# sourmash-bio/sourmash

Measured on AMD Instinct MI355X. Metric: Gbase/s sketched (k=31, scaled=1000), higher is better.
Workload: dtype u64; 1 GPU; C2: sketch synthetic random DNA resident in HBM as ASCII, per GPU 1000 records of 10000000 bases (10000000000 bases, 10000001000 bytes with their separators), k=31 scaled=1000 seed=42; one step = k-mer kernel + radix sort + unique; records_per_gpu=1000, record_len=10000000, bases_per_gpu=10000000000, bytes_per_gpu=10000001000, ksize=31, scaled=1000, unique_hashes_rank0=9998668, unique_hashes_job=9998668, collectives=none (the exchange runs with --full)

## Files before the change

sourmash_amd/csrc/sketch.hip:

```cpp
#include <hip/hip_runtime.h>
#include <stdint.h>
#include <stdlib.h>
#include <utility>
#include "kmer_core.hpp"
#include "sketch_kernel.hpp"
#include "device_api.hpp"

namespace smg {

constexpr int GENERIC_MAX_K = 256;
constexpr int GENERIC_TILE = 4096;

__global__ __launch_bounds__(SK_BLOCK) void sketch_dna_generic_kernel(
    const uint8_t* __restrict__ seq, uint64_t len, uint32_t k, uint64_t seed, uint64_t thr,
    uint64_t* __restrict__ out, unsigned long long* __restrict__ out_count, uint64_t out_cap, uint64_t n_tiles,
    int dense) {
    __shared__ uint8_t s_in[GENERIC_TILE + GENERIC_MAX_K];
    for (uint64_t tile = blockIdx.x; tile < n_tiles; tile += gridDim.x) {
        const uint64_t base = tile * (uint64_t)GENERIC_TILE;
        __syncthreads();
        for (uint32_t i = threadIdx.x; i < GENERIC_TILE + k - 1; i += SK_BLOCK)
            s_in[i] = (base + i < len) ? seq[base + i] : 0;
        __syncthreads();
        for (uint32_t p = threadIdx.x; p < GENERIC_TILE; p += SK_BLOCK) {
            uint8_t fwd[GENERIC_MAX_K], rev[GENERIC_MAX_K];
            bool ok = true;
            for (uint32_t j = 0; j < k; ++j) {
                const uint8_t u = s_in[p + j] & 0xdf;
                uint8_t c;
                switch (u) {
                case 'A': c = 'T'; break;
                case 'C': c = 'G'; break;
                case 'G': c = 'C'; break;
                case 'T': c = 'A'; break;
                default: c = 0; ok = false;
                }
                fwd[j] = u;
                rev[k - 1 - j] = c;
            }
            if (!ok) continue;
            bool use_rev = false;
            for (uint32_t j = 0; j < k; ++j) {
                if (fwd[j] != rev[j]) { use_rev = rev[j] < fwd[j]; break; }
            }
            const uint64_t h = mmh3_h1_bytes(use_rev ? rev : fwd, k, seed);
            if ((h - 1) < thr) {
                if (dense) {
                    if (base + p < out_cap) out[base + p] = h;
                } else {
                    const unsigned long long g = atomicAdd(out_count, 1ull);
                    if (g < out_cap) out[g] = h;
                }
            }
        }
    }
}

__global__ __launch_bounds__(SK_BLOCK) void first_invalid_kernel(const uint8_t* __restrict__ seq, uint64_t len,
                                                                unsigned long long* __restrict__ first) {
    unsigned long long best = ~0ull;
    for (uint64_t i = (uint64_t)blockIdx.x * SK_BLOCK + threadIdx.x; i < len; i += (uint64_t)gridDim.x * SK_BLOCK) {
        const uint8_t u = seq[i] & 0xdf;
        if (!(u == 'A' || u == 'C' || u == 'G' || u == 'T')) { best = i; break; }
    }
    if (best != ~0ull) atomicMin(first, best);
}

constexpr int FAST_MAX_K = SK_FAST_MAX_K;
constexpr int FAST_HERE_K = 64;

static hipError_t sketch_any(const uint8_t* d_seq, uint64_t len, uint32_t k, uint64_t seed, uint64_t thr,
                             uint64_t* d_out, unsigned long long* d_count, uint64_t cap, bool dense,
                             hipStream_t stream) {
    if (len < k || k == 0) return hipSuccess;
    static const bool generic_only = [] { const char* e = getenv("SMG_SKETCH_GENERIC"); return e && *e == '1'; }();
    constexpr uint32_t words_from = (uint32_t)FAST_MAX_K + 1u;
    if (k >= words_from && !generic_only) return sketch_dna_words_launch(d_seq, len, k, seed, thr, d_out, d_count, cap, dense, stream);
    if (!dense && k <= (uint32_t)FAST_MAX_K && !generic_only) {
        const sketch_launch_fn f = k <= (uint32_t)FAST_HERE_K ? sparse_launcher_from<0>(k, std::make_integer_sequence<int, FAST_HERE_K>())
                                                             : sparse_launcher_long(k);
        return f(d_seq, len, seed, thr, d_out, d_count, cap, false, stream);
    }
    if (dense && k <= (uint32_t)FAST_MAX_K && !generic_only)
        return dense_launcher(k)(d_seq, len, seed, thr, d_out, d_count, cap, true, stream);
    if (!generic_only || k > (uint32_t)GENERIC_MAX_K) return sketch_dna_words_launch(d_seq, len, k, seed, thr, d_out, d_count, cap, dense, stream);
    const uint64_t n_tiles = (len + GENERIC_TILE - 1) / GENERIC_TILE;
    const uint64_t max_blocks = 256ull * 8;
    const unsigned grid = (unsigned)(n_tiles < max_blocks ? n_tiles : max_blocks);
    hipLaunchKernelGGL(sketch_dna_generic_kernel, dim3(grid), dim3(SK_BLOCK), 0, stream, d_seq, len, k, seed, thr,
                       d_out, d_count, cap, n_tiles, dense ? 1 : 0);
    return hipGetLastError();
}

hipError_t sketch_dna_launch(const uint8_t* d_seq, uint64_t len, uint32_t k, uint64_t seed, uint64_t thr,
                             uint64_t* d_out, unsigned long long* d_count, uint64_t cap, hipStream_t stream) {
    return sketch_any(d_seq, len, k, seed, thr, d_out, d_count, cap, false, stream);
}

hipError_t kmer_hashes_launch(const uint8_t* d_seq, uint64_t len, uint32_t k, uint64_t seed, uint64_t* d_out,
                              uint64_t n_kmers, hipStream_t stream) {
    return sketch_any(d_seq, len, k, seed, ~0ull, d_out, nullptr, n_kmers, true, stream);
}

hipError_t first_invalid_launch(const uint8_t* d_seq, uint64_t len, unsigned long long* d_first, hipStream_t stream) {
    if (len == 0) return hipSuccess;
    const uint64_t nb = (len + SK_BLOCK - 1) / SK_BLOCK;
    const unsigned grid = (unsigned)(nb < 2048 ? nb : 2048);
    hipLaunchKernelGGL(first_invalid_kernel, dim3(grid), dim3(SK_BLOCK), 0, stream, d_seq, len, d_first);
    return hipGetLastError();
}

}
```

sourmash_amd/csrc/sketch_kernel.hpp:

```cpp
#pragma once
#include <hip/hip_runtime.h>
#include <stdint.h>
#include <utility>
#include "kmer_core.hpp"

namespace smg {

constexpr int SK_BLOCK = 256;
constexpr int SK_FAST_MAX_K = 88;
constexpr int sk_part_size(int first_k_minus_1) { return SK_FAST_MAX_K - first_k_minus_1 < 16 ? SK_FAST_MAX_K - first_k_minus_1 : 16; }
constexpr int SK_OUT_CAP = 2048;

constexpr bool sk_plain_mul(int k, bool dense) {
    if (dense) return k == 1 || k == 5 || k == 8 || k == 25 || k == 28 || k == 81 || k == 82 || k == 84;
    return k == 50 || k == 51;
}

template <int K, int P, bool DENSE>
__global__ __launch_bounds__(SK_BLOCK) void sketch_dna_kernel(
    const uint8_t* __restrict__ seq, uint64_t len, uint64_t seed, uint64_t thr,
    uint64_t* __restrict__ out, unsigned long long* __restrict__ out_count, uint64_t out_cap,
    uint64_t n_tiles, uint32_t skip) {
    using G = LaneGeom<K, P>;
    constexpr int TILE = SK_BLOCK * P;
    constexpr int LANE_RD = ((G::NW + 3) / 4) * 4;
    constexpr int IN_DW = (SK_BLOCK - 1) * (P / 4) + LANE_RD;
    constexpr int IN_CHUNKS = (IN_DW + 3) / 4;
    static_assert(P % 4 == 0, "lane runs must start dword aligned");

    __shared__ __attribute__((aligned(16))) uint32_t s_in[IN_CHUNKS * 4];
    __shared__ uint64_t s_out[SK_OUT_CAP];
    __shared__ unsigned int s_cnt;
    __shared__ unsigned long long s_base;

    const int tid = threadIdx.x;
    if (tid == 0) s_cnt = 0;

    for (uint64_t tile = blockIdx.x; tile < n_tiles; tile += gridDim.x) {
        const uint64_t base = tile * (uint64_t)TILE;
        __syncthreads();
        for (int c = tid; c < IN_CHUNKS; c += SK_BLOCK) {
            const uint64_t off = base + (uint64_t)c * 16;
            uint4 v = make_uint4(0, 0, 0, 0);
            if (off + 16 <= len) {
                v = *reinterpret_cast<const uint4*>(seq + off);
            } else if (off < len) {
                uint32_t w[4] = {0, 0, 0, 0};
                for (uint64_t b = off; b < len; ++b) w[(b - off) >> 2] |= (uint32_t)seq[b] << (8 * ((b - off) & 3));
                v = make_uint4(w[0], w[1], w[2], w[3]);
            }
            if (off == 0 && skip) {
                uint32_t w[4] = {v.x, v.y, v.z, v.w};
                for (uint32_t b = 0; b < skip; ++b) w[b >> 2] &= ~(0xffu << (8 * (b & 3)));
                v = make_uint4(w[0], w[1], w[2], w[3]);
            }
            *reinterpret_cast<uint4*>(&s_in[c * 4]) = v;
        }
        __syncthreads();
        uint32_t raw[LANE_RD];
        const uint4* wp = reinterpret_cast<const uint4*>(&s_in[tid * (P / 4)]);
        static_assert((P / 4) % 4 == 0 || P == 8 || P == 4, "window must stay 16-byte aligned for P=16,32");
#pragma unroll
        for (int i = 0; i < LANE_RD / 4; ++i) {
            if constexpr ((P / 4) % 4 == 0) {
                const uint4 v = wp[i];
                raw[4 * i] = v.x; raw[4 * i + 1] = v.y; raw[4 * i + 2] = v.z; raw[4 * i + 3] = v.w;
            } else {
                const uint32_t* p32 = &s_in[tid * (P / 4) + 4 * i];
                raw[4 * i] = p32[0]; raw[4 * i + 1] = p32[1]; raw[4 * i + 2] = p32[2]; raw[4 * i + 3] = p32[3];
            }
        }
        process_lane<K, P, !DENSE, sk_plain_mul(K, DENSE)>(raw, seed, thr, [&](int o, uint64_t h) {
            if constexpr (DENSE) {
                const uint64_t pos = base + (uint64_t)tid * P + (uint64_t)o - skip;
                if (pos < out_cap) out[pos] = h;
                return;
            }
            const unsigned int idx = atomicAdd(&s_cnt, 1u);
            if (idx < (unsigned)SK_OUT_CAP) {
                s_out[idx] = h;
            } else {
                const unsigned long long g = atomicAdd(out_count, 1ull);
                if (g < out_cap) out[g] = h;
            }
        });
        if constexpr (DENSE) continue;
        __syncthreads();
        const unsigned int cnt = s_cnt;
        if (cnt >= (unsigned)SK_OUT_CAP / 2) {
            const unsigned int n = cnt < (unsigned)SK_OUT_CAP ? cnt : (unsigned)SK_OUT_CAP;
            if (tid == 0) s_base = atomicAdd(out_count, (unsigned long long)n);
            __syncthreads();
            const unsigned long long b = s_base;
            for (unsigned int i = tid; i < n; i += SK_BLOCK)
                if (b + i < out_cap) out[b + i] = s_out[i];
            __syncthreads();
            if (tid == 0) s_cnt = 0;
        }
    }
    if constexpr (DENSE) return;
    __syncthreads();
    const unsigned int cnt = s_cnt;
    if (cnt) {
        const unsigned int n = cnt < (unsigned)SK_OUT_CAP ? cnt : (unsigned)SK_OUT_CAP;
        if (tid == 0) s_base = atomicAdd(out_count, (unsigned long long)n);
        __syncthreads();
        const unsigned long long b = s_base;
        for (unsigned int i = tid; i < n; i += SK_BLOCK)
            if (b + i < out_cap) out[b + i] = s_out[i];
    }
}


typedef hipError_t (*sketch_launch_fn)(const uint8_t*, uint64_t, uint64_t, uint64_t, uint64_t*, unsigned long long*, uint64_t, bool,
                                       hipStream_t);
template <int K>
static hipError_t launch_sparse_k(const uint8_t* d_seq, uint64_t len, uint64_t seed, uint64_t thr, uint64_t* d_out,
                                  unsigned long long* d_count, uint64_t cap, bool, hipStream_t stream) {
    constexpr uint64_t TILE = (uint64_t)SK_BLOCK * 16;
    const uint32_t skip = (uint32_t)((uintptr_t)d_seq & 15);
    d_seq -= skip;
    len += skip;
    const uint64_t n_tiles = (len + TILE - 1) / TILE;
    if (n_tiles == 0) return hipSuccess;
    const uint64_t max_blocks = 256ull * 8;
    const unsigned grid = (unsigned)(n_tiles < max_blocks ? n_tiles : max_blocks);
    hipLaunchKernelGGL((sketch_dna_kernel<K, 16, false>), dim3(grid), dim3(SK_BLOCK), 0, stream, d_seq, len, seed, thr, d_out,
                       d_count, cap, n_tiles, skip);
    return hipGetLastError();
}
template <int K0, int... KS>
static sketch_launch_fn sparse_launcher_from(uint32_t k, std::integer_sequence<int, KS...>) {
    static const sketch_launch_fn table[] = {&launch_sparse_k<K0 + KS + 1>...};
    return table[k - K0 - 1];
}
template <int K>
static hipError_t launch_dense_k(const uint8_t* d_seq, uint64_t len, uint64_t seed, uint64_t thr, uint64_t* d_out,
                                 unsigned long long* d_count, uint64_t cap, bool, hipStream_t stream) {
    constexpr uint64_t TILE = (uint64_t)SK_BLOCK * 16;
    const uint32_t skip = (uint32_t)((uintptr_t)d_seq & 15);
    d_seq -= skip;
    len += skip;
    const uint64_t n_tiles = (len + TILE - 1) / TILE;
    if (n_tiles == 0) return hipSuccess;
    const uint64_t max_blocks = 256ull * 8;
    const unsigned grid = (unsigned)(n_tiles < max_blocks ? n_tiles : max_blocks);
    hipLaunchKernelGGL((sketch_dna_kernel<K, 16, true>), dim3(grid), dim3(SK_BLOCK), 0, stream, d_seq, len, seed, thr, d_out,
                       d_count, cap, n_tiles, skip);
    return hipGetLastError();
}
template <int K0, int... KS>
static sketch_launch_fn dense_launcher_from(uint32_t k, std::integer_sequence<int, KS...>) {
    static const sketch_launch_fn table[] = {&launch_dense_k<K0 + KS + 1>...};
    return table[k - K0 - 1];
}
sketch_launch_fn dense_launcher_0(uint32_t k);
sketch_launch_fn dense_launcher_1(uint32_t k);
sketch_launch_fn dense_launcher_2(uint32_t k);
sketch_launch_fn dense_launcher_3(uint32_t k);
sketch_launch_fn dense_launcher_4(uint32_t k);
sketch_launch_fn dense_launcher_5(uint32_t k);
inline sketch_launch_fn dense_launcher(uint32_t k) {
    switch ((k - 1u) / 16u) {
    case 0: return dense_launcher_0(k);
    case 1: return dense_launcher_1(k);
    case 2: return dense_launcher_2(k);
    case 3: return dense_launcher_3(k);
    case 4: return dense_launcher_4(k);
    default: return dense_launcher_5(k);
    }
}
sketch_launch_fn sparse_launcher_long_0(uint32_t k);
sketch_launch_fn sparse_launcher_long_1(uint32_t k);
inline sketch_launch_fn sparse_launcher_long(uint32_t k) { return k <= 80u ? sparse_launcher_long_0(k) : sparse_launcher_long_1(k); }
static_assert(SK_FAST_MAX_K > 80 && SK_FAST_MAX_K <= 96, "the part tables above");

}
```

sourmash_amd/csrc/kmer_core.hpp:

```cpp
#pragma once
#include "murmur3.hpp"
#include <utility>

namespace smg {

SMG_HD uint32_t perm_b32(uint32_t hi, uint32_t lo, uint32_t sel) {
#if defined(__HIP_DEVICE_COMPILE__)
    return __builtin_amdgcn_perm(hi, lo, sel);
#else
    const uint64_t v = ((uint64_t)hi << 32) | lo;
    uint32_t r = 0;
    for (int i = 0; i < 4; ++i) {
        const uint32_t s = (sel >> (8 * i)) & 0xff;
        uint32_t b;
        if (s < 8) b = (uint32_t)(v >> (8 * s)) & 0xff;
        else if (s == 0x0c) b = 0;
        else b = 0xff;
        r |= b << (8 * i);
    }
    return r;
#endif
}

SMG_HD uint32_t alignbyte_b32(uint32_t hi, uint32_t lo, uint32_t n) {
#if defined(__HIP_DEVICE_COMPILE__)
    return __builtin_amdgcn_alignbyte(hi, lo, n);
#else
    return (uint32_t)((((uint64_t)hi << 32) | lo) >> (8 * n));
#endif
}

SMG_HD bool any_lane(bool p) {
#if defined(__HIP_DEVICE_COMPILE__)
    return __builtin_amdgcn_ballot_w64(p) != 0ull;
#else
    return p;
#endif
}

SMG_HD uint32_t bitselect(uint32_t mask, uint32_t b, uint32_t c) {
#if defined(__HIP_DEVICE_COMPILE__)
    return __builtin_amdgcn_bitop3_b32(mask, b, c, 0xCA);
#else
    return (mask & b) | (~mask & c);
#endif
}

SMG_HD uint32_t opaque(uint32_t x) {
#if defined(__HIP_DEVICE_COMPILE__)
    asm volatile("" : "+v"(x));
#endif
    return x;
}

SMG_HD uint32_t bswap32(uint32_t x) { return perm_b32(0u, x, 0x00010203u); }

constexpr uint32_t LUT_SELF = 'A' | ('C' << 8) | ('T' << 16) | ((uint32_t)'G' << 24);
constexpr uint32_t LUT_COMP = 'T' | ('G' << 8) | ('A' << 16) | ((uint32_t)'C' << 24);

template <int K, int P>
struct LaneGeom {
    static constexpr int NBYTES = P + K - 1;
    static constexpr int NW = (NBYTES + 3) / 4;
    static constexpr int NWK = (K + 3) / 4;
    static constexpr int NCH = (K + 7) / 8;
    static constexpr uint32_t LAST_MASK = (K % 4) ? ((1u << (8 * (K % 4))) - 1u) : 0xffffffffu;
};

constexpr uint32_t rev_sel(int a) {
    return (uint32_t)(a + 3) | ((uint32_t)(a + 2) << 8) | ((uint32_t)(a + 1) << 16) | ((uint32_t)a << 24);
}
constexpr uint32_t rev_sel_partial(int a, int nb) {
    uint32_t s = 0;
    for (int i = 0; i < 4; ++i) {
        const uint32_t b = (i < nb) ? (uint32_t)(a + nb - 1 - i) : 0x0cu;
        s |= b << (8 * i);
    }
    return s;
}

template <int K, int P, int O>
struct PosOps {
    using G = LaneGeom<K, P>;

    template <int D>
    static SMG_HD uint32_t fwd(const uint32_t* U) {
        constexpr int q = (O >> 2) + D, a = O & 3;
        uint32_t v;
        if constexpr (a == 0) v = U[q];
        else if constexpr (q + 1 < G::NW) v = alignbyte_b32(U[q + 1], U[q], a);
        else v = U[q] >> (8 * a);
        if constexpr (D == G::NWK - 1) v &= G::LAST_MASK;
        return v;
    }

    template <int D>
    static SMG_HD uint32_t rev(const uint32_t* C) {
        constexpr int nb = (K - 4 * D) >= 4 ? 4 : (K - 4 * D);
        constexpr int s = O + K - 4 * D - nb;
        constexpr int q = s >> 2, a = s & 3;
        constexpr uint32_t sel = (nb == 4) ? rev_sel(a) : rev_sel_partial(a, nb);
        if constexpr (q + 1 < G::NW) return perm_b32(C[q + 1], C[q], sel);
        else return perm_b32(0u, C[q], sel);
    }

    template <int CH>
    static SMG_HD uint64_t be_chunk(const uint32_t* W) {
        uint64_t v = (uint64_t)bswap32(W[2 * CH]) << 32;
        if constexpr (2 * CH + 1 < G::NWK) v |= bswap32(W[2 * CH + 1]);
        return v;
    }

    template <int CH>
    static SMG_HD uint64_t be_chunk_opaque(const uint32_t* W) {
        uint64_t v = (uint64_t)bswap32(opaque(W[2 * CH])) << 32;
        if constexpr (2 * CH + 1 < G::NWK) v |= bswap32(opaque(W[2 * CH + 1]));
        return v;
    }

    template <int CH>
    static SMG_HD void tie_break(const uint32_t* F, const uint32_t* R, bool& tie, bool& gt) {
        if constexpr (CH < G::NCH) {
            const uint64_t bf = be_chunk_opaque<CH>(F), br = be_chunk_opaque<CH>(R);
            gt = gt || (tie && bf > br);
            tie = tie && (bf == br);
            tie_break<CH + 1>(F, R, tie, gt);
        }
    }

    template <int... D>
    static SMG_HD void build(const uint32_t* U, const uint32_t* C, uint32_t* F, uint32_t* R,
                             std::integer_sequence<int, D...>) {
        ((F[D] = fwd<D>(U)), ...);
        ((R[D] = rev<D>(C)), ...);
    }

    template <bool PLAIN = false>
    static SMG_HD Mmh3Open hash_open(const uint32_t* U, const uint32_t* C, uint64_t seed) {
        uint32_t F[G::NWK], R[G::NWK];
        build(U, C, F, R, std::make_integer_sequence<int, G::NWK>{});
        const uint64_t bf = be_chunk<0>(F), br = be_chunk<0>(R);
        bool gt = bf > br;
        bool tie = bf == br;
        if (G::NCH > 1 && any_lane(tie)) tie_break<1>(F, R, tie, gt);
        uint32_t W[G::NWK];
        const uint32_t m = gt ? 0xffffffffu : 0u;
#pragma unroll
        for (int d = 0; d < G::NWK; ++d) W[d] = bitselect(m, R[d], F[d]);
        return mmh3_open_words<K, PLAIN>(W, seed);
    }
};

SMG_HD uint32_t nonzero_bytes4(uint32_t x) {
    uint32_t t = x | (x >> 4);
    t |= t >> 2;
    t |= t >> 1;
    t &= 0x01010101u;
    return (t * 0x01020408u) >> 24 & 0xfu;
}

SMG_HD uint32_t early_limit(uint64_t thr) {
    const uint32_t thr_hi = (uint32_t)(thr >> 32);
    return thr_hi >= 0xfffffffdu ? 0xffffffffu : thr_hi + 2u;
}
SMG_HD bool early_may_keep(Mmh3Open open, uint32_t lim) { return (uint32_t)(mmh3_close_hi_sum(open) + 1u) <= lim; }

template <int K, int P, bool EARLY, bool PLAIN, class Emit, int... O>
SMG_HD void process_lane_impl(const uint32_t* raw, uint64_t seed, uint64_t thr, Emit&& emit,
                              std::integer_sequence<int, O...>) {
    using G = LaneGeom<K, P>;
    const uint32_t lim = early_limit(thr);
    uint32_t U[G::NW], C[G::NW];
    uint32_t anybad = 0;
#pragma unroll
    for (int i = 0; i < G::NW; ++i) {
        const uint32_t u = raw[i] & 0xdfdfdfdfu;
        const uint32_t code = (u >> 1) & 0x03030303u;
        U[i] = u;
        C[i] = perm_b32(0u, LUT_COMP, code);
        uint32_t bad = perm_b32(0u, LUT_SELF, code) ^ u;
        if (i == G::NW - 1 && (G::NBYTES % 4) != 0)
            bad &= (1u << (8 * (G::NBYTES % 4))) - 1u;
        anybad |= bad;
    }
    uint64_t badlo = 0, badhi = 0, badtop = 0;
    if (anybad != 0) {
#pragma unroll
        for (int i = 0; i < G::NW; ++i) {
            const uint32_t u = U[i];
            const uint32_t code = (u >> 1) & 0x03030303u;
            uint32_t bad = perm_b32(0u, LUT_SELF, code) ^ u;
            if (i == G::NW - 1 && (G::NBYTES % 4) != 0) bad &= (1u << (8 * (G::NBYTES % 4))) - 1u;
            const uint64_t nib = nonzero_bytes4(bad);
            if (4 * i < 64) badlo |= nib << (4 * i);
            else if (4 * i < 128) badhi |= nib << (4 * i - 64);
            else badtop |= nib << (4 * i - 128);
        }
    }
    static_assert(G::NBYTES <= 192 && K <= 128 && P <= 64, "window too long for the 192-bit validity mask");
    (
        [&] {
            const Mmh3Open open = PosOps<K, P, O>::template hash_open<PLAIN>(U, C, seed);
            if constexpr (EARLY) {
                if (!any_lane(early_may_keep(open, lim))) return;
            }
            const uint64_t h = mmh3_close<PLAIN>(open);
            bool ok = (h - 1) < thr;
            if (anybad != 0) {
                uint64_t lo, hi;
                if constexpr (O == 0) { lo = badlo; hi = badhi; }
                else { lo = (badlo >> O) | (badhi << (64 - O)); hi = (badhi >> O) | (badtop << (64 - O)); }
                const uint64_t mlo = K >= 64 ? ~0ull : ((1ull << K) - 1);
                const uint64_t mhi = K >= 128 ? ~0ull : K > 64 ? ((1ull << (K - 64)) - 1) : 0;
                if ((lo & mlo) | (hi & mhi)) ok = false;
            }
            if (ok) emit(O, h);
        }(),
        ...);
}

template <int K, int P, bool EARLY = true, bool PLAIN = false, class Emit>
SMG_HD void process_lane(const uint32_t* raw, uint64_t seed, uint64_t thr, Emit&& emit) {
    process_lane_impl<K, P, EARLY, PLAIN>(raw, seed, thr, static_cast<Emit&&>(emit), std::make_integer_sequence<int, P>{});
}

}
```

Baseline: 324.0 Gbase/s.

## Double-buffer sketch tile staging with async global-to-LDS loads

The sketch kernel now keeps two shared-memory input buffers and issues the next tile's load with global_load_lds into the spare buffer while the current tile is hashed. This is meant to hide HBM load latency behind the hashing work. The per-block output staging shrinks to 1024 entries to make room for the second buffer, and the sparse launch grid grows fourfold. Optional s_memtime instrumentation, compiled in only under SK_TILE_STAMPS, is also added. Risks include higher LDS use lowering occupancy and more frequent flushes of the smaller output buffer.

Measured after the change: 353.7 Gbase/s, median of 6. 1.09x the previous value.

```diff
diff --git a/sourmash_amd/csrc/sketch.hip b/sourmash_amd/csrc/sketch.hip
--- a/sourmash_amd/csrc/sketch.hip
+++ b/sourmash_amd/csrc/sketch.hip
@@ -111,3 +111,14 @@
 }
 
 }
+
+#ifdef SK_TILE_STAMPS
+extern "C" __attribute__((visibility("default"))) int smg_sketch_tile_stamps(unsigned long long* dst, int rows) {
+    unsigned long long* buf = smg::sk_stamp_buffer();
+    if (buf == nullptr || rows < 0 || rows > smg::SK_STAMP_ROWS) return -1;
+    const size_t bytes = (size_t)rows * 4 * sizeof(unsigned long long);
+    if (hipDeviceSynchronize() != hipSuccess) return -1;
+    if (hipMemcpy(dst, buf, bytes, hipMemcpyDeviceToHost) != hipSuccess) return -1;
+    return hipMemset(buf, 0, bytes) == hipSuccess ? 0 : -1;
+}
+#endif
diff --git a/sourmash_amd/csrc/sketch_kernel.hpp b/sourmash_amd/csrc/sketch_kernel.hpp
--- a/sourmash_amd/csrc/sketch_kernel.hpp
+++ b/sourmash_amd/csrc/sketch_kernel.hpp
@@ -10,17 +10,43 @@
 constexpr int SK_FAST_MAX_K = 88;
 constexpr int sk_part_size(int first_k_minus_1) { return SK_FAST_MAX_K - first_k_minus_1 < 16 ? SK_FAST_MAX_K - first_k_minus_1 : 16; }
 constexpr int SK_OUT_CAP = 2048;
+constexpr int SK_TILE_OUT_CAP = 1024;
 
 constexpr bool sk_plain_mul(int k, bool dense) {
     if (dense) return k == 1 || k == 5 || k == 8 || k == 25 || k == 28 || k == 81 || k == 82 || k == 84;
     return k == 50 || k == 51;
 }
+
+#ifdef SK_TILE_STAMPS
+constexpr int SK_STAMP_ROWS = 8192 * 4;
+inline unsigned long long* sk_stamp_buffer() {
+    static unsigned long long* buf = [] {
+        unsigned long long* p = nullptr;
+        if (hipMalloc(&p, SK_STAMP_ROWS * 4 * sizeof(unsigned long long)) != hipSuccess) return (unsigned long long*)nullptr;
+        (void)hipMemset(p, 0, SK_STAMP_ROWS * 4 * sizeof(unsigned long long));
+        return p;
+    }();
+    return buf;
+}
+#define SK_STAMP(t)                                                                        \
+    do {                                                                                   \
+        __builtin_amdgcn_sched_barrier(0);                                                 \
+        asm volatile("s_memtime %0\n\ts_waitcnt lgkmcnt(0)" : "=s"(t) : : "memory");      \
+        __builtin_amdgcn_sched_barrier(0);                                                 \
+    } while (0)
+#define SK_STAMP_PARAM , unsigned long long* __restrict__ stamps
+#define SK_STAMP_ARG , sk_stamp_buffer()
+#else
+#define SK_STAMP(t) do { } while (0)
+#define SK_STAMP_PARAM
+#define SK_STAMP_ARG
+#endif
 
 template <int K, int P, bool DENSE>
 __global__ __launch_bounds__(SK_BLOCK) void sketch_dna_kernel(
     const uint8_t* __restrict__ seq, uint64_t len, uint64_t seed, uint64_t thr,
     uint64_t* __restrict__ out, unsigned long long* __restrict__ out_count, uint64_t out_cap,
-    uint64_t n_tiles, uint32_t skip) {
+    uint64_t n_tiles, uint32_t skip SK_STAMP_PARAM) {
     using G = LaneGeom<K, P>;
     constexpr int TILE = SK_BLOCK * P;
     constexpr int LANE_RD = ((G::NW + 3) / 4) * 4;
@@ -28,18 +54,28 @@
     constexpr int IN_CHUNKS = (IN_DW + 3) / 4;
     static_assert(P % 4 == 0, "lane runs must start dword aligned");
 
-    __shared__ __attribute__((aligned(16))) uint32_t s_in[IN_CHUNKS * 4];
-    __shared__ uint64_t s_out[SK_OUT_CAP];
+    __shared__ __attribute__((aligned(16))) uint32_t s_in[2][IN_CHUNKS * 4];
+    __shared__ uint64_t s_out[SK_TILE_OUT_CAP];
     __shared__ unsigned int s_cnt;
     __shared__ unsigned long long s_base;
 
-    const int tid = threadIdx.x;
-    if (tid == 0) s_cnt = 0;
-
-    for (uint64_t tile = blockIdx.x; tile < n_tiles; tile += gridDim.x) {
-        const uint64_t base = tile * (uint64_t)TILE;
-        __syncthreads();
-        for (int c = tid; c < IN_CHUNKS; c += SK_BLOCK) {
+    if (threadIdx.x == 0) s_cnt = 0;
+
+    auto stage = [&](uint64_t t, uint32_t* dst, uint32_t tid) {
+        const uint64_t base = t * (uint64_t)TILE;
+        if ((t != 0 || skip == 0) && base + (uint64_t)IN_CHUNKS * 16 <= len) {
+            const uint8_t* src = seq + base;
+            const uint32_t wave0 = __builtin_amdgcn_readfirstlane(tid) & ~63u;
+#pragma unroll
+            for (uint32_t r = 0; r < (uint32_t)(IN_CHUNKS + SK_BLOCK - 1) / SK_BLOCK; ++r) {
+                const uint32_t c = r * SK_BLOCK + tid;
+                if (r * SK_BLOCK + wave0 < (uint32_t)IN_CHUNKS && c < (uint32_t)IN_CHUNKS)
+                    __builtin_amdgcn_global_load_lds((const __attribute__((address_space(1))) void*)(src + c * 16u),
+                                                     (__attribute__((address_space(3))) void*)(dst + (r * SK_BLOCK + wave0) * 4u), 16, 0, 0);
+            }
+            return;
+        }
+        for (uint32_t c = tid; c < (uint32_t)IN_CHUNKS; c += SK_BLOCK) {
             const uint64_t off = base + (uint64_t)c * 16;
             uint4 v = make_uint4(0, 0, 0, 0);
             if (off + 16 <= len) {
@@ -54,11 +90,36 @@
                 for (uint32_t b = 0; b < skip; ++b) w[b >> 2] &= ~(0xffu << (8 * (b & 3)));
                 v = make_uint4(w[0], w[1], w[2], w[3]);
             }
-            *reinterpret_cast<uint4*>(&s_in[c * 4]) = v;
-        }
+            *reinterpret_cast<uint4*>(&dst[c * 4]) = v;
+        }
+    };
+    auto flush = [&](unsigned int cnt) {
+        const unsigned int tid = threadIdx.x;
+        const unsigned int n = cnt < (unsigned)SK_TILE_OUT_CAP ? cnt : (unsigned)SK_TILE_OUT_CAP;
+        if (tid == 0) s_base = atomicAdd(out_count, (unsigned long long)n);
         __syncthreads();
+        const unsigned long long b = s_base;
+        if (tid == 0) s_cnt = 0;
+        for (unsigned int i = tid; i < n; i += SK_BLOCK)
+            if (b + i < out_cap) out[b + i] = s_out[i];
+    };
+
+#ifdef SK_TILE_STAMPS
+    unsigned long long t0, t1, t2, t3, t4, sum_wait = 0, sum_stage = 0, sum_hash = 0, sum_flush = 0;
+#endif
+    uint32_t cur = 0;
+    const uint64_t stride = gridDim.x;
+    stage(blockIdx.x, s_in[0], threadIdx.x);
+    for (uint64_t tile = blockIdx.x; tile < n_tiles; tile += stride, cur ^= 1u) {
+        const uint64_t base = tile * (uint64_t)TILE;
+        SK_STAMP(t0);
+        asm volatile("s_waitcnt vmcnt(0)" ::: "memory");
+        __syncthreads();
+        SK_STAMP(t1);
+        const uint32_t tid = opaque(threadIdx.x);
         uint32_t raw[LANE_RD];
-        const uint4* wp = reinterpret_cast<const uint4*>(&s_in[tid * (P / 4)]);
+        const uint32_t* s_cur = s_in[cur];
+        const uint4* wp = reinterpret_cast<const uint4*>(&s_cur[tid * (P / 4)]);
         static_assert((P / 4) % 4 == 0 || P == 8 || P == 4, "window must stay 16-byte aligned for P=16,32");
 #pragma unroll
         for (int i = 0; i < LANE_RD / 4; ++i) {
@@ -66,10 +127,12 @@
                 const uint4 v = wp[i];
                 raw[4 * i] = v.x; raw[4 * i + 1] = v.y; raw[4 * i + 2] = v.z; raw[4 * i + 3] = v.w;
             } else {
-                const uint32_t* p32 = &s_in[tid * (P / 4) + 4 * i];
+                const uint32_t* p32 = &s_cur[tid * (P / 4) + 4 * i];
                 raw[4 * i] = p32[0]; raw[4 * i + 1] = p32[1]; raw[4 * i + 2] = p32[2]; raw[4 * i + 3] = p32[3];
             }
         }
+        if (tile + stride < n_tiles) stage(tile + stride, s_in[cur ^ 1u], tid);
+        SK_STAMP(t2);
         process_lane<K, P, !DENSE, sk_plain_mul(K, DENSE)>(raw, seed, thr, [&](int o, uint64_t h) {
             if constexpr (DENSE) {
                 const uint64_t pos = base + (uint64_t)tid * P + (uint64_t)o - skip;
@@ -77,38 +140,34 @@
                 return;
             }
             const unsigned int idx = atomicAdd(&s_cnt, 1u);
-            if (idx < (unsigned)SK_OUT_CAP) {
+            if (idx < (unsigned)SK_TILE_OUT_CAP) {
                 s_out[idx] = h;
             } else {
                 const unsigned long long g = atomicAdd(out_count, 1ull);
                 if (g < out_cap) out[g] = h;
             }
         });
-        if constexpr (DENSE) continue;
-        __syncthreads();
-        const unsigned int cnt = s_cnt;
-        if (cnt >= (unsigned)SK_OUT_CAP / 2) {
-            const unsigned int n = cnt < (unsigned)SK_OUT_CAP ? cnt : (unsigned)SK_OUT_CAP;
-            if (tid == 0) s_base = atomicAdd(out_count, (unsigned long long)n);
+        SK_STAMP(t3);
+        if constexpr (!DENSE) {
             __syncthreads();
-            const unsigned long long b = s_base;
-            for (unsigned int i = tid; i < n; i += SK_BLOCK)
-                if (b + i < out_cap) out[b + i] = s_out[i];
-            __syncthreads();
-            if (tid == 0) s_cnt = 0;
-        }
+            const unsigned int cnt = s_cnt;
+            if (cnt >= (unsigned)SK_TILE_OUT_CAP / 2) flush(cnt);
+        }
+        SK_STAMP(t4);
+#ifdef SK_TILE_STAMPS
+        sum_wait += t1 - t0; sum_stage += t2 - t1; sum_hash += t3 - t2; sum_flush += t4 - t3;
+#endif
     }
+#ifdef SK_TILE_STAMPS
+    if ((threadIdx.x & 63) == 0 && stamps != nullptr && blockIdx.x * 4u + (threadIdx.x >> 6) < (unsigned)SK_STAMP_ROWS) {
+        unsigned long long* row = stamps + ((size_t)blockIdx.x * 4 + (threadIdx.x >> 6)) * 4;
+        row[0] += sum_wait; row[1] += sum_stage; row[2] += sum_hash; row[3] += sum_flush;
+    }
+#endif
     if constexpr (DENSE) return;
     __syncthreads();
     const unsigned int cnt = s_cnt;
-    if (cnt) {
-        const unsigned int n = cnt < (unsigned)SK_OUT_CAP ? cnt : (unsigned)SK_OUT_CAP;
-        if (tid == 0) s_base = atomicAdd(out_count, (unsigned long long)n);
-        __syncthreads();
-        const unsigned long long b = s_base;
-        for (unsigned int i = tid; i < n; i += SK_BLOCK)
-            if (b + i < out_cap) out[b + i] = s_out[i];
-    }
+    if (cnt) flush(cnt);
 }
 
 
@@ -123,10 +182,10 @@
     len += skip;
     const uint64_t n_tiles = (len + TILE - 1) / TILE;
     if (n_tiles == 0) return hipSuccess;
-    const uint64_t max_blocks = 256ull * 8;
+    const uint64_t max_blocks = 256ull * 32;
     const unsigned grid = (unsigned)(n_tiles < max_blocks ? n_tiles : max_blocks);
     hipLaunchKernelGGL((sketch_dna_kernel<K, 16, false>), dim3(grid), dim3(SK_BLOCK), 0, stream, d_seq, len, seed, thr, d_out,
-                       d_count, cap, n_tiles, skip);
+                       d_count, cap, n_tiles, skip SK_STAMP_ARG);
     return hipGetLastError();
 }
 template <int K0, int... KS>
@@ -146,7 +205,7 @@
     const uint64_t max_blocks = 256ull * 8;
     const unsigned grid = (unsigned)(n_tiles < max_blocks ? n_tiles : max_blocks);
     hipLaunchKernelGGL((sketch_dna_kernel<K, 16, true>), dim3(grid), dim3(SK_BLOCK), 0, stream, d_seq, len, seed, thr, d_out,
-                       d_count, cap, n_tiles, skip);
+                       d_count, cap, n_tiles, skip SK_STAMP_ARG);
     return hipGetLastError();
 }
 template <int K0, int... KS>
```

## Stage case-fold and complement once per tile in shared memory

Applied to the files above, without the earlier changes.

For sparse kernels at most k values, the case-folded input and its complement are computed once per 16-byte chunk during the cooperative tile load and stored in a second shared buffer. A block-wide dirty flag then lets lanes skip per-lane validity checks when the whole tile is clean. This removes the redundant per-lane recomputation of the overlapping window's fold, complement and bad-base tests. In exchange it doubles shared memory for the input tile, adds a second LDS read per lane, and adds a racy shared flag write.

Result: faster. 324.9 Gbase/s before, 331.5 Gbase/s after (median of 6 runs) (+2.0%).

```diff
diff --git a/sourmash_amd/csrc/kmer_core.hpp b/sourmash_amd/csrc/kmer_core.hpp
--- a/sourmash_amd/csrc/kmer_core.hpp
+++ b/sourmash_amd/csrc/kmer_core.hpp
@@ -224,4 +224,106 @@
     process_lane_impl<K, P, EARLY, PLAIN>(raw, seed, thr, static_cast<Emit&&>(emit), std::make_integer_sequence<int, P>{});
 }
 
-}
+
+template <int K, int P, int BLOCK>
+struct TileGeom {
+    using G = LaneGeom<K, P>;
+    static constexpr int TILE = BLOCK * P;
+    static constexpr int LANE_RD = ((G::NW + 3) / 4) * 4;
+    static constexpr int IN_DW = (BLOCK - 1) * (P / 4) + LANE_RD;
+    static constexpr int IN_CHUNKS = (IN_DW + 3) / 4;
+};
+
+SMG_HD void load_chunk(const uint8_t* seq, uint64_t off, uint64_t len, uint32_t skip, uint32_t* w) {
+    w[0] = w[1] = w[2] = w[3] = 0;
+    if (off + 16 <= len) {
+#if defined(__HIP_DEVICE_COMPILE__)
+        const uint4 v = *reinterpret_cast<const uint4*>(seq + off);
+        w[0] = v.x; w[1] = v.y; w[2] = v.z; w[3] = v.w;
+#else
+        for (int b = 0; b < 16; ++b) w[b >> 2] |= (uint32_t)seq[off + b] << (8 * (b & 3));
+#endif
+    } else if (off < len) {
+        for (uint64_t b = off; b < len; ++b) w[(b - off) >> 2] |= (uint32_t)seq[b] << (8 * ((b - off) & 3));
+    }
+    if (off == 0 && skip) {
+        for (uint32_t b = 0; b < skip; ++b) w[b >> 2] &= ~(0xffu << (8 * (b & 3)));
+    }
+}
+
+SMG_HD uint32_t stage_chunk(uint32_t* w, uint32_t* c) {
+    uint32_t anybad = 0;
+#pragma unroll
+    for (int j = 0; j < 4; ++j) {
+        const uint32_t u = w[j] & 0xdfdfdfdfu;
+        const uint32_t code = (u >> 1) & 0x03030303u;
+        w[j] = u;
+        c[j] = perm_b32(0u, LUT_COMP, code);
+        anybad |= perm_b32(0u, LUT_SELF, code) ^ u;
+    }
+    return anybad;
+}
+
+template <int K, int P>
+SMG_HD void lane_bad_bits(const uint32_t* U, uint64_t& badlo, uint64_t& badhi, uint64_t& badtop) {
+    using G = LaneGeom<K, P>;
+    static_assert(G::NBYTES <= 192 && K <= 128 && P <= 64, "window too long for the 192-bit validity mask");
+#pragma unroll
+    for (int i = 0; i < G::NW; ++i) {
+        const uint32_t u = U[i];
+        const uint32_t code = (u >> 1) & 0x03030303u;
+        uint32_t bad = perm_b32(0u, LUT_SELF, code) ^ u;
+        if (i == G::NW - 1 && (G::NBYTES % 4) != 0) bad &= (1u << (8 * (G::NBYTES % 4))) - 1u;
+        const uint64_t nib = nonzero_bytes4(bad);
+        if (4 * i < 64) badlo |= nib << (4 * i);
+        else if (4 * i < 128) badhi |= nib << (4 * i - 64);
+        else badtop |= nib << (4 * i - 128);
+    }
+}
+
+template <int K, int P, bool EARLY, bool PLAIN, class Emit, int... O>
+SMG_HD void lane_positions(const uint32_t* U, const uint32_t* C, uint32_t anybad, uint64_t badlo, uint64_t badhi, uint64_t badtop,
+                           uint64_t seed, uint64_t thr, Emit&& emit, std::integer_sequence<int, O...>) {
+    const uint32_t lim = early_limit(thr);
+    (
+        [&] {
+            const Mmh3Open open = PosOps<K, P, O>::template hash_open<PLAIN>(U, C, seed);
+            if constexpr (EARLY) {
+                if (!any_lane(early_may_keep(open, lim))) return;
+            }
+            const uint64_t h = mmh3_close<PLAIN>(open);
+            bool ok = (h - 1) < thr;
+            if (anybad != 0) {
+                uint64_t lo, hi;
+                if constexpr (O == 0) { lo = badlo; hi = badhi; }
+                else { lo = (badlo >> O) | (badhi << (64 - O)); hi = (badhi >> O) | (badtop << (64 - O)); }
+                const uint64_t mlo = K >= 64 ? ~0ull : ((1ull << K) - 1);
+                const uint64_t mhi = K >= 128 ? ~0ull : K > 64 ? ((1ull << (K - 64)) - 1) : 0;
+                if ((lo & mlo) | (hi & mhi)) ok = false;
+            }
+            if (ok) emit(O, h);
+        }(),
+        ...);
+}
+
+template <int K, int P, bool EARLY = true, bool PLAIN = false, class Emit>
+SMG_HD void process_lane_staged(const uint32_t* U, const uint32_t* C, bool dirty, uint64_t seed, uint64_t thr, Emit&& emit) {
+    using G = LaneGeom<K, P>;
+    uint32_t anybad = 0;
+    uint64_t badlo = 0, badhi = 0, badtop = 0;
+    if (dirty) {
+#pragma unroll
+        for (int i = 0; i < G::NW; ++i) {
+            const uint32_t u = U[i];
+            uint32_t bad = perm_b32(0u, LUT_SELF, (u >> 1) & 0x03030303u) ^ u;
+            if (i == G::NW - 1 && (G::NBYTES % 4) != 0)
+                bad &= (1u << (8 * (G::NBYTES % 4))) - 1u;
+            anybad |= bad;
+        }
+        if (anybad != 0) lane_bad_bits<K, P>(U, badlo, badhi, badtop);
+    }
+    lane_positions<K, P, EARLY, PLAIN>(U, C, anybad, badlo, badhi, badtop, seed, thr, static_cast<Emit&&>(emit),
+                                       std::make_integer_sequence<int, P>{});
+}
+
+}
diff --git a/sourmash_amd/csrc/sketch_kernel.hpp b/sourmash_amd/csrc/sketch_kernel.hpp
--- a/sourmash_amd/csrc/sketch_kernel.hpp
+++ b/sourmash_amd/csrc/sketch_kernel.hpp
@@ -15,20 +15,21 @@
     if (dense) return k == 1 || k == 5 || k == 8 || k == 25 || k == 28 || k == 81 || k == 82 || k == 84;
     return k == 50 || k == 51;
 }
+constexpr bool sk_staged(int k) { return k > 11 && k != 18 && k != 20 && k != 30; }
 
 template <int K, int P, bool DENSE>
 __global__ __launch_bounds__(SK_BLOCK) void sketch_dna_kernel(
     const uint8_t* __restrict__ seq, uint64_t len, uint64_t seed, uint64_t thr,
     uint64_t* __restrict__ out, unsigned long long* __restrict__ out_count, uint64_t out_cap,
     uint64_t n_tiles, uint32_t skip) {
-    using G = LaneGeom<K, P>;
-    constexpr int TILE = SK_BLOCK * P;
-    constexpr int LANE_RD = ((G::NW + 3) / 4) * 4;
-    constexpr int IN_DW = (SK_BLOCK - 1) * (P / 4) + LANE_RD;
-    constexpr int IN_CHUNKS = (IN_DW + 3) / 4;
+    using T = TileGeom<K, P, SK_BLOCK>;
+    constexpr int TILE = T::TILE, LANE_RD = T::LANE_RD, IN_CHUNKS = T::IN_CHUNKS;
+    constexpr bool STAGED = !DENSE && sk_staged(K);
     static_assert(P % 4 == 0, "lane runs must start dword aligned");
 
     __shared__ __attribute__((aligned(16))) uint32_t s_in[IN_CHUNKS * 4];
+    __shared__ __attribute__((aligned(16))) uint32_t s_comp[STAGED ? IN_CHUNKS * 4 : 4];
+    __shared__ unsigned int s_dirty;
     __shared__ uint64_t s_out[SK_OUT_CAP];
     __shared__ unsigned int s_cnt;
     __shared__ unsigned long long s_base;
@@ -38,9 +39,20 @@
 
     for (uint64_t tile = blockIdx.x; tile < n_tiles; tile += gridDim.x) {
         const uint64_t base = tile * (uint64_t)TILE;
+        if constexpr (STAGED) {
+            if (tid == 0) s_dirty = 0;
+        }
         __syncthreads();
         for (int c = tid; c < IN_CHUNKS; c += SK_BLOCK) {
             const uint64_t off = base + (uint64_t)c * 16;
+            if constexpr (STAGED) {
+                uint32_t w[4], cw[4];
+                load_chunk(seq, off, len, skip, w);
+                if (stage_chunk(w, cw)) s_dirty = 1;
+                *reinterpret_cast<uint4*>(&s_comp[c * 4]) = make_uint4(cw[0], cw[1], cw[2], cw[3]);
+                *reinterpret_cast<uint4*>(&s_in[c * 4]) = make_uint4(w[0], w[1], w[2], w[3]);
+                continue;
+            }
             uint4 v = make_uint4(0, 0, 0, 0);
             if (off + 16 <= len) {
                 v = *reinterpret_cast<const uint4*>(seq + off);
@@ -70,7 +82,7 @@
                 raw[4 * i] = p32[0]; raw[4 * i + 1] = p32[1]; raw[4 * i + 2] = p32[2]; raw[4 * i + 3] = p32[3];
             }
         }
-        process_lane<K, P, !DENSE, sk_plain_mul(K, DENSE)>(raw, seed, thr, [&](int o, uint64_t h) {
+        auto emit = [&](int o, uint64_t h) {
             if constexpr (DENSE) {
                 const uint64_t pos = base + (uint64_t)tid * P + (uint64_t)o - skip;
                 if (pos < out_cap) out[pos] = h;
@@ -83,7 +95,21 @@
                 const unsigned long long g = atomicAdd(out_count, 1ull);
                 if (g < out_cap) out[g] = h;
             }
-        });
+        };
+        if constexpr (STAGED) {
+            static_assert(!STAGED || P == 16, "the staged form reads whole 16-byte groups");
+            uint32_t comp[LANE_RD];
+            const uint4* cp = reinterpret_cast<const uint4*>(&s_comp[tid * (P / 4)]);
+#pragma unroll
+            for (int i = 0; i < LANE_RD / 4; ++i) {
+                const uint4 v = cp[i];
+                comp[4 * i] = v.x; comp[4 * i + 1] = v.y; comp[4 * i + 2] = v.z; comp[4 * i + 3] = v.w;
+            }
+            const bool dirty = __builtin_amdgcn_readfirstlane(s_dirty) != 0;
+            process_lane_staged<K, P, true, sk_plain_mul(K, false)>(raw, comp, dirty, seed, thr, emit);
+        } else {
+            process_lane<K, P, !DENSE, sk_plain_mul(K, DENSE)>(raw, seed, thr, emit);
+        }
         if constexpr (DENSE) continue;
         __syncthreads();
         const unsigned int cnt = s_cnt;
```
